# Quantco/tabmat

Hardware: AMD Instinct MI355X
Metric: SplitMatrix.sandwich GFLOP/s + effective HBM GB/s, 10M×1k mixed (higher is better)
Workload: dtype f64; 1 GPU; SplitMatrix.sandwich: dense128 + csr512@5% + cats(256,96,32), 10000000 rows/GPU, p=1024, float64 (BASELINE configs[3]); rows_per_gpu=10000000, p=1024, launch=eager, collective=none

## Files before the change

### tabmat_amd/csrc/cat.hip

```cpp
#include <algorithm>

#include "common.hpp"
#include "reduce.hpp"

namespace tmh {

__global__ void fill_i32_kernel(int32_t *p, int64_t n, int32_t v) {
    int64_t i = (int64_t)blockIdx.x * blockDim.x + threadIdx.x;
    if (i < n) p[i] = v;
}

__global__ void scatter_iota_i32_kernel(int32_t *map, const int32_t *cols, int64_t n_cols) {
    int64_t i = (int64_t)blockIdx.x * blockDim.x + threadIdx.x;
    if (i < n_cols) map[cols[i]] = (int32_t)i;
}

int build_col_map(int32_t *map, int64_t m, const int32_t *cols, int64_t n_cols, hipStream_t st) {
    if (m > 0) {
        hipLaunchKernelGGL(fill_i32_kernel, dim3((unsigned)ceil_div(m, 256)), dim3(256), 0, st, map,
                           m, -1);
        TM_LAUNCH_CHECK();
    }
    if (n_cols > 0) {
        hipLaunchKernelGGL(scatter_iota_i32_kernel, dim3((unsigned)ceil_div(n_cols, 256)),
// ... 5 lines not shown

template <typename F, bool TWO>
__global__ __launch_bounds__(1024) void hist_lds_kernel(
    const int32_t *__restrict__ ci, const int32_t *__restrict__ cj, const F *__restrict__ w,
    const int32_t *__restrict__ rows, int64_t n_iter, int64_t rows_per_block, int drop_i,
    int drop_j, int i_ncol, int j_ncol, int ti, const int32_t *__restrict__ col_map,
    F *__restrict__ ws, int64_t stride) {
    extern __shared__ __attribute__((aligned(16))) unsigned char smem_raw[];
    lds_acc_t *bins = reinterpret_cast<lds_acc_t *>(smem_raw);
    const int part = blockIdx.y;
    const int i0 = part * ti;
    const int i1 = min(i0 + ti, i_ncol);
    const int nbins = TWO ? (i1 - i0) * j_ncol : (i1 - i0);
    for (int b = threadIdx.x; b < nbins; b += blockDim.x) bins[b] = 0.0;
    __syncthreads();

    const int64_t t0 = (int64_t)blockIdx.x * rows_per_block;
    const int64_t t1 = min(t0 + rows_per_block, n_iter);
    int64_t tbeg = t0;
    if (!TWO && rows == nullptr && (t0 & 3) == 0 &&
        ((reinterpret_cast<uintptr_t>(ci) | reinterpret_cast<uintptr_t>(w)) & 15) == 0) {
        typedef int i4 __attribute__((ext_vector_type(4)));
        const int64_t nvec = (t1 - t0) / 4;
        for (int64_t q = threadIdx.x; q < nvec; q += blockDim.x) {
            const int64_t k = t0 + q * 4;
            const i4 cc = *reinterpret_cast<const i4 *>(ci + k);
            F ww[4];
#pragma unroll
            for (int e = 0; e < 4; ++e) ww[e] = w[k + e];
#pragma unroll
            for (int e = 0; e < 4; ++e) {
                const int c = cc[e] - drop_i;
                if (c >= i0 && c < i1 && !(col_map && col_map[c] < 0)) atomic_add(&bins[c - i0], (lds_acc_t)ww[e]);
            }
        }
        tbeg = t0 + nvec * 4;
    }
    for (int64_t t = tbeg + threadIdx.x; t < t1; t += blockDim.x) {
        const int64_t k = rows ? (int64_t)rows[t] : t;
        const int c = ci[k] - drop_i;
        if (c < i0 || c >= i1) continue;
        if (TWO) {
            const int c2 = cj[k] - drop_j;
            if (c2 < 0) continue;
            atomic_add(&bins[(c - i0) * j_ncol + c2], (lds_acc_t)w[k]);
        } else {
            if (col_map && col_map[c] < 0) continue;
            atomic_add(&bins[c - i0], (lds_acc_t)w[k]);
        }
    }
    __syncthreads();
    F *dst = ws + ((int64_t)part * gridDim.x + blockIdx.x) * stride;
    for (int b = threadIdx.x; b < nbins; b += blockDim.x) dst[b] = (F)bins[b];
}

template <typename F, bool TWO>
__global__ __launch_bounds__(256) void hist_global_kernel(
    const int32_t *__restrict__ ci, const int32_t *__restrict__ cj, const F *__restrict__ w,
    const int32_t *__restrict__ rows, int64_t n_iter, int drop_i, int drop_j, int j_ncol,
    const int32_t *__restrict__ col_map, F *__restrict__ out) {
    const int64_t stride = (int64_t)gridDim.x * blockDim.x;
    for (int64_t t = (int64_t)blockIdx.x * blockDim.x + threadIdx.x; t < n_iter; t += stride) {
        const int64_t k = rows ? (int64_t)rows[t] : t;
        const int c = ci[k] - drop_i;
        if (c < 0) continue;
        if (TWO) {
// ... 1203 lines not shown
    cs->total = off;
    return TM_OK;
}

template <typename F>
static int run_multi_cat_dense(const void *const *h_codes, const int64_t *h_ncols,
                               const int32_t *h_drop, int n_cats, int64_t n, const F *d, const F *M,
                               int64_t m, int order_f, F *out, hipStream_t st,
                               const int32_t *rows = nullptr, int64_t n_rows = 0) {
    CatSet cs;
    int rc = make_catset(h_codes, h_ncols, h_drop, n_cats, &cs);
    if (rc) return rc;
    const int64_t total = (int64_t)cs.total * m;
    if (total == 0) return TM_OK;
    if (rows != nullptr) n = n_rows;
    if (n == 0) {
        TM_HIP(hipMemsetAsync(out, 0, sizeof(F) * (size_t)total, st));
        return TM_OK;
    }
    {
        constexpr int VEC = MCW_VEC;
        constexpr int TJW = 16 * VEC;
        const size_t tile_b = ((sizeof(lds_acc_t) * (size_t)cs.total * TJW + 15) / 16) * 16;
        const size_t lds_w = tile_b + (size_t)16 * MCW_RS * (sizeof(F) + (size_t)n_cats * sizeof(int));
        if (!order_f && n_cats <= 8 && m >= VEC && m % VEC == 0 &&
            (reinterpret_cast<uintptr_t>(M) & 15) == 0 && lds_w <= 150 * 1024 &&
            (int64_t)cs.total * TJW * (int64_t)sizeof(lds_acc_t) < (1ll << 30)) {
            const int64_t n_parts = ceil_div(m, TJW);
            const int64_t stride = (int64_t)cs.total * TJW;
            int64_t nblk = std::max<int64_t>(1, tune("catdense_rounds", 1) * NUM_CU / n_parts);
            nblk = std::min<int64_t>(nblk, std::max<int64_t>(1, ceil_div(n, 4096)));
            const int64_t rpb = ceil_div(ceil_div(n, nblk), MCW_RS) * MCW_RS;
            nblk = ceil_div(n, rpb);
            const size_t tmp_bytes = ((sizeof(F) * (size_t)(n_parts * stride) + 255) / 256) * 256;
            void *wsv = nullptr;
            rc = get_workspace(tmp_bytes + sizeof(F) * (size_t)(n_parts * nblk * stride) + 256, &wsv, st);
            if (rc) return rc;
            F *tmp = reinterpret_cast<F *>(wsv);
            F *ws = reinterpret_cast<F *>(reinterpret_cast<char *>(wsv) + tmp_bytes);
            auto gow = [&](auto kern) -> int {
                TM_HIP(hipFuncSetAttribute(reinterpret_cast<const void *>(kern),
                                           hipFuncAttributeMaxDynamicSharedMemorySize, (int)lds_w));
                prof_begin(st);
                const int nw_dflt = (sizeof(F) == 8 && tile_b > 64 * 1024) ? 8 : 16;
                const int nw = (int)std::min<int64_t>(16, std::max<int64_t>(4, tune("catdense_waves", nw_dflt)));
                hipLaunchKernelGGL(kern, dim3((unsigned)nblk, (unsigned)n_parts), dim3(nw * 64), lds_w, st,
                                   cs, d, M, n, m, rpb, ws, stride, rows, wg_log_ptr());
                prof_end(st);
                TM_LAUNCH_CHECK();
                return TM_OK;
            };
            if (n_cats == 1) rc = gow(&multi_cat_dense_wide_kernel<F, 1>);
            else if (n_cats == 2) rc = gow(&multi_cat_dense_wide_kernel<F, 2>);
            else if (n_cats == 3) rc = gow(&multi_cat_dense_wide_kernel<F, 3>);
            else if (n_cats == 4) rc = gow(&multi_cat_dense_wide_kernel<F, 4>);
            else if (n_cats == 5) rc = gow(&multi_cat_dense_wide_kernel<F, 5>);
            else if (n_cats == 6) rc = gow(&multi_cat_dense_wide_kernel<F, 6>);
            else if (n_cats == 7) rc = gow(&multi_cat_dense_wide_kernel<F, 7>);
            else rc = gow(&multi_cat_dense_wide_kernel<F, 8>);
            if (rc) return rc;
            rc = launch_reduce_partials<F>(ws, stride, (int)nblk, (int)n_parts, tmp, n_parts * stride,
                                           false, st);
            if (rc) return rc;
            hipLaunchKernelGGL((multi_cat_untile_kernel<F>), dim3((unsigned)ceil_div(total, 256)),
                               dim3(256), 0, st, tmp, (int64_t)cs.total, m, TJW, out);
            TM_LAUNCH_CHECK();
            return TM_OK;
        }
    }
    if (rows != nullptr) {
        set_error("multi_cat_dense: the row-list form needs the wide-load path");
        return TM_EUNSUPPORTED;
    }
    int TJ = 64;
    while (TJ > 1 && sizeof(lds_acc_t) * (size_t)cs.total * TJ > HIST_LDS_MAX) TJ >>= 1;
    while (TJ > 1 && TJ / 2 >= m) TJ >>= 1;
    if (sizeof(lds_acc_t) * (size_t)cs.total * TJ > HIST_LDS_MAX) {
        set_error("multi_cat_dense: %d stacked categories exceed the LDS tile", cs.total);
        return TM_EUNSUPPORTED;
    }
    const int64_t n_parts = ceil_div(m, TJ);
    const int64_t stride = (int64_t)cs.total * TJ;
    const size_t lds = sizeof(lds_acc_t) * (size_t)stride;
    int64_t nblk = std::max<int64_t>(1, NUM_CU / n_parts);
    nblk = std::min<int64_t>(nblk, std::max<int64_t>(1, ceil_div(n, 4096)));
    const int64_t rpb = ceil_div(n, nblk);
    nblk = ceil_div(n, rpb);
    const size_t tmp_bytes = ((sizeof(F) * (size_t)(n_parts * stride) + 255) / 256) * 256;
    void *wsv = nullptr;
    rc = get_workspace(tmp_bytes + sizeof(F) * (size_t)(n_parts * nblk * stride) + 256, &wsv, st);
    if (rc) return rc;
    F *tmp = reinterpret_cast<F *>(wsv);
    F *ws = reinterpret_cast<F *>(reinterpret_cast<char *>(wsv) + tmp_bytes);
    auto go = [&](auto kern) -> int {
        if (lds > 48 * 1024)
            TM_HIP(hipFuncSetAttribute(reinterpret_cast<const void *>(kern),
                                       hipFuncAttributeMaxDynamicSharedMemorySize, (int)lds));
        prof_begin(st);
        hipLaunchKernelGGL(kern, dim3((unsigned)nblk, (unsigned)n_parts), dim3(1024), lds, st, cs, d,
                           M, n, m, rpb, ws, stride);
// ... 132 lines not shown
}

template <typename F>
static int run_multi_cat_sparse_ent(const void *const *h_codes, const int64_t *h_ncols, const int32_t *h_drop,
                                    int n_cats, int64_t n, const F *d, const F *vals, const unsigned short *meta,
                                    const unsigned *bstart, int64_t mk, F *out, hipStream_t st,
                                    const unsigned *packed = nullptr, int64_t n_slots = 0) {
    CatSet cs;
    int rc = make_catset(h_codes, h_ncols, h_drop, n_cats, &cs);
    if (rc) return rc;
    const int64_t total = (int64_t)cs.total * mk;
    if (total == 0) return TM_OK;
    if (n == 0) {
        TM_HIP(hipMemsetAsync(out, 0, sizeof(F) * (size_t)total, st));
        return TM_OK;
    }
    TM_REQUIRE(mk % 16 == 0 && n_cats >= 1 && n_cats <= 8, "kernel columns in groups of 16, 1 .. 8 categoricals");
    TM_REQUIRE(n < (1ll << 28), "at most 2^28 - 1 rows per block");
    constexpr int GC = 32;
    const int64_t stride = (int64_t)cs.total * GC;
    const size_t lds = ((sizeof(lds_acc_t) * (size_t)cs.total * (GC + 1) + 15) / 16) * 16;
    if (lds > HIST_LDS_MAX) {
        set_error("multi_cat_sparse_ent: %d stacked categories exceed the LDS tile", cs.total);
        return TM_EUNSUPPORTED;
    }
    const int nw = (int)std::min<int64_t>(16, std::max<int64_t>(4, tune("catsparse_waves", 16)));
    const int n_groups = (int)(mk / 16);
    const int n_pairs = (n_groups + 1) / 2;
    const int64_t n_slabs = ceil_div(n, 64);
    int64_t nblk = std::max<int64_t>(1, tune("catsparse_rounds", 1) * NUM_CU / n_pairs);
    nblk = std::min<int64_t>(nblk, n_slabs);
    const int64_t spb = ceil_div(n_slabs, nblk);
    nblk = ceil_div(n_slabs, spb);
    const size_t tmp_bytes = ((sizeof(F) * (size_t)(n_pairs * stride) + 255) / 256) * 256;
    void *wsv = nullptr;
    rc = get_workspace(tmp_bytes + sizeof(F) * (size_t)((int64_t)n_pairs * nblk * stride) + 256, &wsv, st);
    if (rc) return rc;
    F *tmp = reinterpret_cast<F *>(wsv);
    F *ws = reinterpret_cast<F *>(reinterpret_cast<char *>(wsv) + tmp_bytes);
    auto kern = n_cats == 1   ? &multi_cat_sparse_ent_kernel<F, 1>
                : n_cats == 2 ? &multi_cat_sparse_ent_kernel<F, 2>
                : n_cats == 3 ? &multi_cat_sparse_ent_kernel<F, 3>
                : n_cats == 4 ? &multi_cat_sparse_ent_kernel<F, 4>
                : n_cats == 5 ? &multi_cat_sparse_ent_kernel<F, 5>
                : n_cats == 6 ? &multi_cat_sparse_ent_kernel<F, 6>
                : n_cats == 7 ? &multi_cat_sparse_ent_kernel<F, 7>
                              : &multi_cat_sparse_ent_kernel<F, 8>;
    TM_REQUIRE(packed == nullptr || (n_cats <= 3 && cs.total < 1023), "packed codes: at most 3 categoricals, 1022 levels");
    const int ncw = packed != nullptr ? 1 : n_cats;
    const size_t lds_staged = lds + (size_t)nw * 64 * (sizeof(F) + 4 * (size_t)ncw);
    const double fill = (double)n_slots / ((double)std::max(n_groups, 1) * (double)n_slabs);
    if (tune("catsparse_staged", 1) != 0 && lds_staged <= 156 * 1024 &&
        fill >= (double)tune("catsparse_staged_fill", 44)) {
        using KS = void (*)(CatSet, const F *, const F *, const unsigned short *, const unsigned *, int, int64_t, int64_t,
                            int64_t, F *, int64_t, const unsigned *, int);
        KS ks = nullptr;
        if (packed != nullptr) {
            ks = n_cats == 1 ? &multi_cat_sparse_ent_staged_kernel<F, 1, true>
                 : n_cats == 2 ? &multi_cat_sparse_ent_staged_kernel<F, 2, true>
                               : &multi_cat_sparse_ent_staged_kernel<F, 3, true>;
        } else {
            ks = n_cats == 1   ? &multi_cat_sparse_ent_staged_kernel<F, 1, false>
                 : n_cats == 2 ? &multi_cat_sparse_ent_staged_kernel<F, 2, false>
                 : n_cats == 3 ? &multi_cat_sparse_ent_staged_kernel<F, 3, false>
                 : n_cats == 4 ? &multi_cat_sparse_ent_staged_kernel<F, 4, false>
                 : n_cats == 5 ? &multi_cat_sparse_ent_staged_kernel<F, 5, false>
                 : n_cats == 6 ? &multi_cat_sparse_ent_staged_kernel<F, 6, false>
                 : n_cats == 7 ? &multi_cat_sparse_ent_staged_kernel<F, 7, false>
                               : &multi_cat_sparse_ent_staged_kernel<F, 8, false>;
        }
        if (lds_staged > 48 * 1024)
            TM_HIP(hipFuncSetAttribute(reinterpret_cast<const void *>(ks),
                                       hipFuncAttributeMaxDynamicSharedMemorySize, (int)lds_staged));
        prof_begin(st);
        hipLaunchKernelGGL(ks, dim3((unsigned)nblk, (unsigned)n_pairs), dim3(nw * 64), lds_staged, st, cs, d, vals,
                           meta, bstart, n_groups, n, n_slabs, spb, ws, stride, packed, (int)lds);
        prof_end(st);
        TM_LAUNCH_CHECK();
    } else {
        if (lds > 48 * 1024)
            TM_HIP(hipFuncSetAttribute(reinterpret_cast<const void *>(kern),
                                       hipFuncAttributeMaxDynamicSharedMemorySize, (int)lds));
        prof_begin(st);
        hipLaunchKernelGGL(kern, dim3((unsigned)nblk, (unsigned)n_pairs), dim3(nw * 64), lds, st, cs, d, vals, meta,
                           bstart, n_groups, n, n_slabs, spb, ws, stride, packed);
        prof_end(st);
        TM_LAUNCH_CHECK();
    }
    rc = launch_reduce_partials<F>(ws, stride, (int)nblk, n_pairs, tmp, (int64_t)n_pairs * stride, false, st);
    if (rc) return rc;
    hipLaunchKernelGGL((multi_cat_untile_kernel<F>), dim3((unsigned)ceil_div(total, 256)), dim3(256), 0, st, tmp,
                       (int64_t)cs.total, mk, GC, out);
    TM_LAUNCH_CHECK();
    return TM_OK;
}

}

using namespace tmh;

#define TM_CHECK_COMMON(nn) \
    TM_REQUIRE((nn) >= 0, "negative size")

extern "C" {

int tm_cat_transpose_matvec_f32(const int32_t *codes, int64_t n, int64_t n_cols, int drop_first,
                                const float *v, const int32_t *rows, int64_t n_rows,
                                const int32_t *cols, int64_t n_cols_sel, float *out, void *stream) {
    TM_CHECK_COMMON(n);
    return run_cat_tmv<float>(codes, n, n_cols, drop_first, v, rows, n_rows, cols, n_cols_sel, out,
                              as_stream(stream));
}
int tm_cat_transpose_matvec_f64(const int32_t *codes, int64_t n, int64_t n_cols, int drop_first,
                                const double *v, const int32_t *rows, int64_t n_rows,
                                const int32_t *cols, int64_t n_cols_sel, double *out,
                                void *stream) {
    TM_CHECK_COMMON(n);
    return run_cat_tmv<double>(codes, n, n_cols, drop_first, v, rows, n_rows, cols, n_cols_sel,
                               out, as_stream(stream));
}

int tm_cat_matvec_f32(const int32_t *codes, int64_t n, int64_t n_cols, int drop_first,
                      const float *v, const int32_t *cols, int64_t n_cols_sel, float *out,
                      void *stream) {
    TM_CHECK_COMMON(n);
    return run_cat_matvec<float>(codes, n, n_cols, drop_first, v, cols, n_cols_sel, out,
                                 as_stream(stream));
// ... 298 lines not shown
```

### tabmat_amd/csrc/reduce.hpp

```cpp
#pragma once
#include "common.hpp"

namespace tmh {

template <typename F, bool ACCUMULATE, int NW>
__global__ __launch_bounds__(NW * 64) void reduce_partials_kernel(const F *__restrict__ ws,
                                                                  int64_t stride, int nb,
                                                                  F *__restrict__ out,
                                                                  int64_t out_elems) {
    __shared__ double red[NW][64];
    const int lane = threadIdx.x & 63;
    const int wave = threadIdx.x >> 6;
    const int64_t e = (int64_t)blockIdx.x * 64 + lane;
    const int part = blockIdx.y;
    double acc = 0.0;
    if (e < stride) {
        const F *p = ws + ((int64_t)part * nb) * stride + e;
        for (int b = wave; b < nb; b += NW) acc += (double)p[(int64_t)b * stride];
    }
    red[wave][lane] = acc;
    __syncthreads();
    if (wave == 0 && e < stride) {
        const int64_t o = (int64_t)part * stride + e;
        if (o < out_elems) {
// ... 2 lines not shown
            for (int w = 0; w < NW; w += 4)
                s += (red[w][lane] + red[w + 1][lane]) + (red[w + 2][lane] + red[w + 3][lane]);
            if (ACCUMULATE)
                out[o] += (F)s;
            else
                out[o] = (F)s;
        }
    }
}

template <typename F>
inline int launch_reduce_partials(const F *ws, int64_t stride, int nb, int n_parts, F *out,
                                  int64_t out_elems, bool accumulate, hipStream_t st) {
    dim3 grid((unsigned)ceil_div(stride, 64), (unsigned)n_parts);
    const bool small = (int64_t)grid.x * grid.y < 1024 && nb > 16;
    if (small) {
        if (accumulate)
            hipLaunchKernelGGL((reduce_partials_kernel<F, true, 16>), grid, dim3(1024), 0, st, ws,
                               stride, nb, out, out_elems);
        else
            hipLaunchKernelGGL((reduce_partials_kernel<F, false, 16>), grid, dim3(1024), 0, st, ws,
                               stride, nb, out, out_elems);
    } else if (accumulate) {
        hipLaunchKernelGGL((reduce_partials_kernel<F, true, 4>), grid, dim3(256), 0, st, ws, stride,
                           nb, out, out_elems);
    } else {
        hipLaunchKernelGGL((reduce_partials_kernel<F, false, 4>), grid, dim3(256), 0, st, ws, stride,
                           nb, out, out_elems);
    }
    TM_LAUNCH_CHECK();
    return TM_OK;
}

__global__ void fill_i32_kernel(int32_t *p, int64_t n, int32_t v);
__global__ void scatter_iota_i32_kernel(int32_t *map, const int32_t *cols, int64_t n_cols);

int build_col_map(int32_t *map, int64_t m, const int32_t *cols, int64_t n_cols, hipStream_t st);

}
```

### tabmat_amd/csrc/sparse_blocks.hip

```cpp
#include <algorithm>

#include "common.hpp"
#include "reduce.hpp"

namespace tmh {

constexpr int KB_WAVES = 16;
constexpr int KB_TS = 128;

template <typename F>
__global__ void blocks_assemble_kernel(const F *__restrict__ tiles, int n_out, F *__restrict__ out) {
    const int j = blockIdx.x * blockDim.x + threadIdx.x;
    const int i = blockIdx.y;
    if (i >= n_out || j >= n_out) return;
    const int hi = max(i, j), lo = min(i, j);
    const int I = hi / KB_TS, J = lo / KB_TS;
    const int part = I * (I + 1) / 2 + J;
    out[(int64_t)i * n_out + j] = tiles[(int64_t)part * KB_TS * KB_TS + (hi % KB_TS) * KB_TS + (lo % KB_TS)];
}

constexpr int KB_FLAG_REP_A = 1 << 16;
constexpr int KB_FLAG_REP_B = 1 << 17;

template <typename F, bool U8, bool D12 = false>
__global__ __launch_bounds__(KB_WAVES * 64) void sparse_sandwich_blocks_kernel(
    const F *__restrict__ data, const int32_t *__restrict__ ind, const int32_t *__restrict__ cptr,
    int64_t n, int64_t nnz1, const int32_t *__restrict__ blocks, const int4 *__restrict__ wg_tab,
    const F *__restrict__ d, int max_nb, F *__restrict__ ws, WgLogBuf *__restrict__ wglog) {
    constexpr int TS = KB_TS;
    const unsigned long long t_begin = wg_log_begin(wglog);
    extern __shared__ __attribute__((aligned(16))) unsigned char smem_raw[];
    lds_acc_t *tile = reinterpret_cast<lds_acc_t *>(smem_raw);
    const int4 w = wg_tab[2 * blockIdx.x], x = wg_tab[2 * blockIdx.x + 1];
    const int part = __builtin_amdgcn_readfirstlane(w.x), slot = __builtin_amdgcn_readfirstlane(w.y);
    const int b0 = __builtin_amdgcn_readfirstlane(w.z), b1 = __builtin_amdgcn_readfirstlane(w.w);
    const int bfull = __builtin_amdgcn_readfirstlane(x.x);
    int wfull = __builtin_amdgcn_readfirstlane(x.y);
    {
        const int nwv = (int)(blockDim.x >> 6);
        if (nwv != KB_WAVES) {
            wfull = (wfull * nwv + KB_WAVES / 2) / KB_WAVES;
            if (bfull > b0) wfull = max(wfull, 1);
            if (b1 > bfull) wfull = min(wfull, nwv - 1);
            if (bfull == b0) wfull = 0;
            if (b1 == bfull) wfull = nwv;
        }
    }
    int I = (int)((sqrtf(8.0f * (float)part + 1.0f) - 1.0f) * 0.5f);
    while ((I + 1) * (I + 2) / 2 <= part) ++I;
    while (I * (I + 1) / 2 > part) --I;
    const int J = part - I * (I + 1) / 2;
    const int i0 = I * TS, j0 = J * TS;
// ... 131 lines not shown
        };
        auto run_tile = [&](auto diag_c) {
            if (wave < wfull) run_list(diag_c, std::true_type{}, b0, bfull, 0, wfull);
            else run_list(diag_c, std::false_type{}, bfull, b1, wfull, (int)(blockDim.x >> 6) - wfull);
        };
        if (I == J) run_tile(std::true_type{});
        else run_tile(std::false_type{});
    }
    __syncthreads();
    if (threadIdx.x == 0) wg_log_end(wglog, t_begin, WG_K2);
    F *dst = ws + ((int64_t)part * max_nb + slot) * (TS * TS);
    for (int b = threadIdx.x; b < TS * TS; b += blockDim.x) {
        const int r = b / TS, c = b % TS;
        dst[b] = (F)tile[r * TS + (c ^ ((r & 15) << 3))];
    }
}

template <typename F, bool U8 = false, bool D12 = false>
static int run_sparse_sandwich_blocks(const F *data, const int32_t *ind, const int32_t *cptr, int64_t n,
                                      int64_t m, int64_t nnz, const int32_t *blocks, const int32_t *wg_tab,
                                      int n_wg, int max_nb, const F *d, F *out, hipStream_t st) {
    if (m == 0) return TM_OK;
    if (n == 0 || nnz == 0 || n_wg == 0) {
        TM_HIP(hipMemsetAsync(out, 0, sizeof(F) * (size_t)(m * m), st));
        return TM_OK;
    }
    constexpr int TS = KB_TS;
    const int nchunk = (int)ceil_div(m, TS);
    const int n_parts = nchunk * (nchunk + 1) / 2;
    TM_REQUIRE(nnz < (1ll << 31) && n < (1ll << 29), "sparse block too large for the block-list sandwich");
    TM_REQUIRE(!D12 || n < (1ll << 24), "12-byte block descriptors hold 24 bits of row");
    TM_REQUIRE(max_nb >= 1 && n_wg >= 1, "empty workgroup table");
    const size_t lds = sizeof(lds_acc_t) * (size_t)(TS * TS);
    const size_t tmp_bytes = (sizeof(F) * (size_t)n_parts * TS * TS + 255) / 256 * 256;
    const size_t ws_bytes = sizeof(F) * (size_t)n_parts * (size_t)max_nb * TS * TS;
    void *wsv = nullptr;
    int rc = get_workspace(tmp_bytes + ws_bytes + 256, &wsv, st);
    if (rc) return rc;
    F *tmp = reinterpret_cast<F *>(wsv);
    F *ws = reinterpret_cast<F *>(reinterpret_cast<char *>(wsv) + tmp_bytes);
    TM_HIP(hipMemsetAsync(ws, 0, ws_bytes, st));
    auto kern = &sparse_sandwich_blocks_kernel<F, U8, D12>;
    TM_HIP(hipFuncSetAttribute(reinterpret_cast<const void *>(kern),
                               hipFuncAttributeMaxDynamicSharedMemorySize, (int)lds));
    prof_begin(st);
    const int kb_waves = (int)std::min<int64_t>(KB_WAVES, std::max<int64_t>(2, tune("k2b_waves", KB_WAVES)));
    hipLaunchKernelGGL(kern, dim3((unsigned)n_wg), dim3(kb_waves * 64), lds, st, data, ind, cptr, n, nnz - 1,
                       blocks, reinterpret_cast<const int4 *>(wg_tab), d,
                       max_nb, ws, wg_log_ptr());
    prof_end(st);
    TM_LAUNCH_CHECK();
    rc = launch_reduce_partials<F>(ws, (int64_t)TS * TS, max_nb, n_parts, tmp, (int64_t)n_parts * TS * TS,
                                   false, st);
    if (rc) return rc;
    hipLaunchKernelGGL((blocks_assemble_kernel<F>), dim3((unsigned)ceil_div(m, 64), (unsigned)m), dim3(64),
                       0, st, tmp, (int)m, out);
    TM_LAUNCH_CHECK();
    return TM_OK;
}

}

extern "C" {

int tm_sparse_sandwich_blocks_f32(const float *cm_data, const int32_t *cm_indices, const int32_t *cptr,
                                  int64_t n, int64_t m, int64_t nnz, const int32_t *blocks,
                                  const int32_t *wg_tab, int n_wg, int max_nb, const float *d, float *out,
                                  void *stream) {
    return tmh::run_sparse_sandwich_blocks<float>(cm_data, cm_indices, cptr, n, m, nnz, blocks, wg_tab, n_wg,
                                                  max_nb, d, out, tmh::as_stream(stream));
}
int tm_sparse_sandwich_blocks_f64(const double *cm_data, const int32_t *cm_indices, const int32_t *cptr,
                                  int64_t n, int64_t m, int64_t nnz, const int32_t *blocks,
                                  const int32_t *wg_tab, int n_wg, int max_nb, const double *d, double *out,
                                  void *stream) {
    return tmh::run_sparse_sandwich_blocks<double>(cm_data, cm_indices, cptr, n, m, nnz, blocks, wg_tab, n_wg,
                                                   max_nb, d, out, tmh::as_stream(stream));
}

int tm_sparse_sandwich_blocks_u8_f32(const float *cm_data, const uint8_t *cm_col8, const int32_t *cptr,
                                     int64_t n, int64_t m, int64_t nnz, const int32_t *blocks,
                                     const int32_t *wg_tab, int n_wg, int max_nb, const float *d, float *out,
                                     void *stream) {
    return tmh::run_sparse_sandwich_blocks<float, true>(cm_data, reinterpret_cast<const int32_t *>(cm_col8), cptr, n, m,
                                                        nnz, blocks, wg_tab, n_wg, max_nb, d, out,
                                                        tmh::as_stream(stream));
}
int tm_sparse_sandwich_blocks_u8_f64(const double *cm_data, const uint8_t *cm_col8, const int32_t *cptr,
                                     int64_t n, int64_t m, int64_t nnz, const int32_t *blocks,
                                     const int32_t *wg_tab, int n_wg, int max_nb, const double *d, double *out,
                                     void *stream) {
// ... 24 lines not shown
```

### tabmat_amd/csrc/sparse_ent.hip

```cpp
#include "common.hpp"
#include "reduce.hpp"

namespace tmh {

constexpr int EN_R = 64;
constexpr int EN_C = 16;
constexpr int EN_NW = 16;
constexpr int EN_THREADS = EN_NW * 64;
constexpr int EN_W = 128;
constexpr int EN_B = 16;
constexpr int EN_SB = 64;

template <typename F>
struct EnLds {
    static constexpr int ROWB = EN_W * (int)sizeof(F);
    static constexpr int SLABB = EN_R * ROWB;
    static constexpr int SCR_OFF = ROWB + 2 * SLABB;
    static constexpr int CS_OFF = SCR_OFF + EN_NW * EN_SB * 16;
    static constexpr int TOTAL = CS_OFF + EN_NW * EN_C * (int)sizeof(double);
};

constexpr int EN_CVGPR = 24;
#define EN_LD "40"

// ... 286 lines not shown
#endif
    }
    while (w < ns) end_slab();
    wait_loads(std::integral_constant<int, 0>{});
#if defined(EN_PROF)
    if (prof != nullptr && lane == 0) {
        long long *o = prof + (((int64_t)blockIdx.z * gridDim.y + blockIdx.y) * gridDim.x + blockIdx.x) * (EN_NW * 8) + wave * 8;
        o[0] = pt_a; o[1] = pt_p; o[2] = pt_x; o[3] = pt_b; o[4] = pt_bar; o[5] = pt_n; o[6] = clock64() - pt_start; o[7] = ns;
    }
#endif

    if (active) {
        F *dst = ws + (((int64_t)blockIdx.y * gridDim.x + blockIdx.x) * n_groups + group) * (EN_C * EN_W);
        static_for<EN_C>([&](auto jc) {
            constexpr int j = decltype(jc)::value;
            if constexpr (sizeof(F) == 8) {
                const u4 o = u4{en_read_acc<4 * j>(), en_read_acc<4 * j + 1>(), en_read_acc<4 * j + 2>(),
                                en_read_acc<4 * j + 3>()};
                *reinterpret_cast<u4 *>(dst + j * EN_W + 2 * lane) = o;
            } else {
                typedef unsigned u2 __attribute__((ext_vector_type(2)));
                const u2 o = u2{en_read_acc<2 * j>(), en_read_acc<2 * j + 1>()};
                *reinterpret_cast<u2 *>(dst + j * EN_W + 2 * lane) = o;
            }
        });
        if constexpr (CSUM) {
            if (blockIdx.y == 0 && lane < EN_C)
                ws_csum[(int64_t)blockIdx.x * (n_groups * EN_C) + group * EN_C + lane] = (F)cs_lds[lane];
        }
    }
}

template <typename F>
__global__ void en_untile_kernel(const F *__restrict__ tmp, int64_t m, int64_t nB, F *__restrict__ out) {
    const int64_t e = (int64_t)blockIdx.x * blockDim.x + threadIdx.x;
    if (e >= m * nB) return;
    const int64_t i = e / nB, j = e % nB;
    out[e] = tmp[((j / EN_W) * m + i) * EN_W + (j % EN_W)];
}

template <typename F>
__global__ void en_csum_kernel(const F *__restrict__ part, int nblk, int64_t m, F *__restrict__ csum) {
    const int64_t c = (int64_t)blockIdx.x * blockDim.x + threadIdx.x;
    if (c >= m) return;
    double a = 0.0;
    for (int b = 0; b < nblk; ++b) a += (double)part[(int64_t)b * m + c];
    csum[c] = (F)a;
}

template <typename F>
static int run_csr_dense_ent(const F *vals, const uint16_t *meta, const uint32_t *bstart, int64_t n, int64_t m,
                             const F *B, int64_t r, const F *d, F *out, F *colsum, hipStream_t st) {
    const int64_t nB = r;
    const int64_t total = m * nB;
    if (total == 0) return TM_OK;
    constexpr int VEC = 16 / (int)sizeof(F);
    if ((reinterpret_cast<uintptr_t>(B) & 15) != 0 || r % VEC != 0 || nB < VEC) {
        set_error("tm_csr_dense_sandwich_ent: B must be C-ordered with 16-byte aligned rows");
        return TM_EUNSUPPORTED;
    }
    if (m % EN_C != 0) {
        set_error("tm_csr_dense_sandwich_ent: m must be a multiple of tm_ent_group_cols()");
        return TM_EINVAL;
    }
    if (n >= (1ll << 28)) {
        set_error("tm_csr_dense_sandwich_ent: at most 2^28 - 1 rows per block (work in row parts)");
        return TM_EUNSUPPORTED;
    }
    const int64_t n_slabs = ceil_div(n, EN_R);
    const int n_groups = (int)(m / EN_C);
    const int n_parts = (int)ceil_div(nB, EN_W);
    const int nz = (int)ceil_div(n_groups, EN_NW);
    const bool want_csum = colsum != nullptr;
    if (n_slabs == 0) {
        TM_HIP(hipMemsetAsync(out, 0, sizeof(F) * (size_t)total, st));
        if (want_csum) TM_HIP(hipMemsetAsync(colsum, 0, sizeof(F) * (size_t)m, st));
        return TM_OK;
    }
    int64_t nblk = std::max<int64_t>(1, tune("ent_rounds", 1) * NUM_CU / ((int64_t)n_parts * nz));
    nblk = std::min<int64_t>(nblk, n_slabs);
    const int64_t spb = ceil_div(n_slabs, nblk);
    nblk = ceil_div(n_slabs, spb);
    const int64_t stride = m * EN_W;
    const size_t tmp_bytes = (sizeof(F) * (size_t)(n_parts * stride) + 255) / 256 * 256;
    const size_t part_bytes = (sizeof(F) * (size_t)((int64_t)n_parts * nblk * stride) + 255) / 256 * 256;
    const size_t csum_bytes = ((want_csum ? sizeof(F) * (size_t)(nblk * m) : 0) + 255) / 256 * 256 + 256;
    void *wsv = nullptr;
    int rc = get_workspace(tmp_bytes + part_bytes + csum_bytes + 256, &wsv, st);
    if (rc) return rc;
    F *tmp = reinterpret_cast<F *>(wsv);
    F *ws = reinterpret_cast<F *>(reinterpret_cast<char *>(wsv) + tmp_bytes);
    F *ws_csum = reinterpret_cast<F *>(reinterpret_cast<char *>(wsv) + tmp_bytes + part_bytes);
    const size_t lds = (size_t)EnLds<F>::TOTAL;
    auto kern = want_csum ? &csr_dense_ent_kernel<F, true> : &csr_dense_ent_kernel<F, false>;
    TM_HIP(hipFuncSetAttribute(reinterpret_cast<const void *>(kern),
                               hipFuncAttributeMaxDynamicSharedMemorySize, (int)lds));
    prof_begin(st);
    hipLaunchKernelGGL(kern, dim3((unsigned)nblk, (unsigned)n_parts, (unsigned)nz), dim3(EN_THREADS), lds, st,
                       vals, meta, bstart, n_groups, n_slabs, spb, B, n, r, (int)nB, d, ws, ws_csum,
                       reinterpret_cast<long long *>((uintptr_t)tune("ent_prof", 0)));
    prof_end(st);
    TM_LAUNCH_CHECK();
    rc = launch_reduce_partials<F>(ws, stride, (int)nblk, n_parts, tmp, n_parts * stride, false, st);
    if (rc) return rc;
    hipLaunchKernelGGL((en_untile_kernel<F>), dim3((unsigned)ceil_div(total, 256)), dim3(256), 0, st, tmp, m,
                       nB, out);
    TM_LAUNCH_CHECK();
    if (want_csum) {
        hipLaunchKernelGGL((en_csum_kernel<F>), dim3((unsigned)ceil_div(m, 256)), dim3(256), 0, st, ws_csum,
                           (int)nblk, m, colsum);
        TM_LAUNCH_CHECK();
    }
    return TM_OK;
}

}

extern "C" {
int tm_ent_rows(void) { return tmh::EN_R; }
int tm_ent_group_cols(void) { return tmh::EN_C; }
int tm_ent_batch_slots(void) { return tmh::EN_B; }

int tm_csr_dense_sandwich_ent_f32(const float *vals, const uint16_t *meta, const uint32_t *bstart, int64_t n,
                                  int64_t m, const float *B, int64_t r, const float *d, float *out,
                                  float *colsum, void *stream) {
    return tmh::run_csr_dense_ent<float>(vals, meta, bstart, n, m, B, r, d, out, colsum, tmh::as_stream(stream));
}
int tm_csr_dense_sandwich_ent_f64(const double *vals, const uint16_t *meta, const uint32_t *bstart, int64_t n,
                                  int64_t m, const double *B, int64_t r, const double *d, double *out,
                                  double *colsum, void *stream) {
    return tmh::run_csr_dense_ent<double>(vals, meta, bstart, n, m, B, r, d, out, colsum, tmh::as_stream(stream));
}
}
```

### tabmat_amd/csrc/syrk_i8.hip

```cpp
#include <algorithm>
#include <cmath>

#include "common.hpp"

#if defined(I8_NO_SB)
#define I8_SB
#else
#define I8_SB __builtin_amdgcn_sched_barrier(0)
#endif
#if defined(I8_TRACE)
#define I8_STAMP(k)                                                                                     \
    do {                                                                                                \
        if (blockIdx.x == 0 && lane == 0 && trace_it >= 8 && trace_it < 12)                             \
            trace_buf[((trace_it - 8) * 4 + wave) * 8 + (k)] = __builtin_readcyclecounter();            \
    } while (0)
#else
#define I8_STAMP(k)
#endif
namespace tmh {

constexpr int I8_W = 128;
constexpr int I8_T = 36;
constexpr int I8_ND = 5;
constexpr int I8_WLO = 2;
// ... 156 lines not shown
    }
    sigma[i] = s;
    rscale[i] = r;
}

template <bool CSUM, bool CEN, bool TV = false>
__global__ __launch_bounds__(I8_THREADS) __attribute__((amdgpu_waves_per_eu(1, 1)))
void syrk_i8_kernel(const double *__restrict__ X, int64_t ldx, int64_t n, int64_t m, const double *__restrict__ d,
                    const double *__restrict__ sigma, const I8Info *__restrict__ info, int n_items,
                    unsigned *__restrict__ counter, double *__restrict__ part, double *__restrict__ colsum,
                    const double *__restrict__ center, const double *__restrict__ v = nullptr,
                    double *__restrict__ xtv = nullptr) {
    if (info->flag != 0) return;
    __shared__ __attribute__((aligned(16))) unsigned char planes[I8_PLANES];
    __shared__ __attribute__((aligned(16))) unsigned char raw[3 * I8_RAWBUF];
    __shared__ double dl[3 * I8_HS];
    __shared__ double vl[TV ? 3 * I8_HS : 1];
    __shared__ unsigned slot_mem[4];
    unsigned *slot = slot_mem;
#if defined(I8_TRACE)
    unsigned long long *trace_buf = reinterpret_cast<unsigned long long *>(reinterpret_cast<char *>(counter) - 256 + 2560);
    int trace_it = 0;
#endif

    const int tid = threadIdx.x;
    const int lane = tid & 63;
    const int wave = __builtin_amdgcn_readfirstlane(tid >> 6);
    const int cl = lane & 15, rq = lane >> 4;

    unsigned idL = blockIdx.x;
    int hL = 0;
    unsigned idNext;
    if (tid == 0) *slot = gridDim.x + atomicAdd(counter, 1u);
    __syncthreads();
    idNext = __builtin_amdgcn_readfirstlane(*slot);
    bool pending = false;

    using C0 = std::integral_constant<int, 0>;
    using C1 = std::integral_constant<int, 1>;
    double dreg = 0.0, vreg = 0.0;
    const int dma_voff = lane * 2 < m ? lane * 16 : 0x7ffffff0;
    auto issue_half = [&](int rb) -> unsigned {
        const unsigned id = idL;
        const int64_t tb = (int64_t)id * I8_ITEM_ROWS + (int64_t)hL * I8_HS;
        const int64_t left = min((n - tb) * ldx * 8, (int64_t)I8_HS * ldx * 8);
        const uint64_t xb = (uint64_t)(uintptr_t)(X + tb * ldx);
        const unsigned xlo = __builtin_amdgcn_readfirstlane((unsigned)xb);
        const unsigned xhi = __builtin_amdgcn_readfirstlane((unsigned)(xb >> 32));
        const unsigned nbytes = __builtin_amdgcn_readfirstlane(
            left <= 0 ? 0u : (left > 0xFFFFFFFFll ? 0xFFFFFFFFu : (unsigned)left));
        const i8_rsrc_t rs = i8_rsrc(reinterpret_cast<const void *>((uintptr_t)(((uint64_t)xhi << 32) | xlo)), nbytes);
        if (wave == 0 && lane < I8_HS) dreg = tb + lane < n ? d[tb + lane] : 0.0;
        if constexpr (TV) {
            if (wave == 0 && lane < I8_HS) vreg = tb + lane < n ? v[tb + lane] : 0.0;
        }
#if !defined(I8_ABLATE_NO_DMA)
#pragma unroll
        for (int j = 0; j < 8; ++j)
            i8_dma16(rs, raw + rb * I8_RAWBUF + (8 * wave + j) * I8_RAWSTR, (int)((8 * wave + j) * ldx * 8) + dma_voff);
#endif
        if (++hL == 2 * I8_CPI) {
            hL = 0;
            idL = idNext;
            if (tid == 0) *slot = gridDim.x + atomicAdd(counter, 1u);
            pending = true;
        }
// ... 412 lines not shown

int run_syrk_i8_panel(const double *X, int64_t ldx, int64_t n, int64_t m, const double *d, const double *colmax,
                      double *out, int64_t ldo, double *colsum, int *history, hipStream_t st, const double *center,
                      const double *v, double *xtv) {
    TM_REQUIRE((v == nullptr) == (xtv == nullptr), "v and xtv go together");
    TM_REQUIRE(v == nullptr || colsum == nullptr, "X' d and X' v are not built into one int8 kernel");
    TM_REQUIRE(n >= 0 && m >= 0, "negative shape");
    TM_REQUIRE(ldx >= m && ldo >= m, "row strides");
    TM_REQUIRE(m == 0 || syrk_co_ok(X, m), "the int8 syrk takes a 16-byte aligned C-ordered f64 block of <= 128 columns");
    if (m == 0) return TM_OK;
    if (n == 0) {
        TM_HIP(hipMemset2DAsync(out, sizeof(double) * (size_t)ldo, 0, sizeof(double) * (size_t)m, (size_t)m, st));
        if (colsum) TM_HIP(hipMemsetAsync(colsum, 0, sizeof(double) * (size_t)m, st));
        if (xtv) TM_HIP(hipMemsetAsync(xtv, 0, sizeof(double) * (size_t)m, st));
        return TM_OK;
    }
    if (colsum) TM_HIP(hipMemsetAsync(colsum, 0, sizeof(double) * (size_t)m, st));
    if (xtv) TM_HIP(hipMemsetAsync(xtv, 0, sizeof(double) * (size_t)m, st));
    const int64_t n_items64 = ceil_div(n, I8_ITEM_ROWS);
    TM_REQUIRE(n_items64 < (1ll << 31), "too many rows");
    const int n_items = (int)n_items64;
    const int grid = (int)std::max<int64_t>(1, std::min<int64_t>(n_items, tune("i8_grid", NUM_CU)));
    const size_t part_bytes = sizeof(double) * (size_t)grid * I8_T * 256;
    const size_t own_bytes = (4096 + part_bytes + 255) / 256 * 256;
    void *wsv = nullptr;
    int rc = get_workspace(own_bytes + syrk_co_ws_bytes(), &wsv, st);
    if (rc) return rc;
    char *wb = reinterpret_cast<char *>(wsv);
    I8Info *info = reinterpret_cast<I8Info *>(wb);
    unsigned *counter = reinterpret_cast<unsigned *>(wb + 256);
    double *sigma = reinterpret_cast<double *>(wb + 512);
    double *rscale = reinterpret_cast<double *>(wb + 512 + 1024);
    double *part = reinterpret_cast<double *>(wb + 4096);
    TM_HIP(hipMemsetAsync(wb, 0, 4096 + part_bytes, st));
    const int sgrid = (int)std::min<int64_t>(4 * NUM_CU, ceil_div(n, 1024));
    hipLaunchKernelGGL(i8_screen_kernel, dim3((unsigned)sgrid), dim3(256), 0, st, d, n, info);
    hipLaunchKernelGGL(i8_scale_kernel, dim3(1), dim3(I8_W), 0, st, colmax, (int)m, n, info, sigma, rscale, history);
    TM_LAUNCH_CHECK();
    prof_begin(st);
    auto go = [&](auto kern) {
        hipLaunchKernelGGL(kern, dim3((unsigned)grid), dim3(I8_THREADS), 0, st, X, ldx, n, m, d, sigma, info, n_items,
                           counter, part, colsum, center, v, xtv);
    };
    if (v) {
        if (center) go(syrk_i8_kernel<false, true, true>);
        else go(syrk_i8_kernel<false, false, true>);
    } else if (center) {
        if (colsum) go(syrk_i8_kernel<true, true>);
        else go(syrk_i8_kernel<false, true>);
    } else {
        if (colsum) go(syrk_i8_kernel<true, false>);
        else go(syrk_i8_kernel<false, false>);
    }
    prof_end(st);
    TM_LAUNCH_CHECK();
    hipLaunchKernelGGL(syrk_i8_finish_kernel, dim3(I8_T, 4), dim3(64, 16), 0, st, part, grid, (int)m, rscale, info,
                       out, ldo);
    hipLaunchKernelGGL(i8_envelope_kernel, dim3(1), dim3(I8_W), 0, st, out, ldo, colmax, (int)m, n, info, history);
    TM_LAUNCH_CHECK();
    prof_hold(true);
    rc = run_syrk_co_flagged(X, ldx, n, m, d, out, ldo, colsum, &info->flag, wb + own_bytes, st, center, v, xtv);
    prof_hold(false);
    if (rc == TM_OK && history != nullptr) {
        hipLaunchKernelGGL(i8_record_diag_kernel, dim3(1), dim3(I8_W), 0, st, out, ldo, (int)m, history);
        TM_LAUNCH_CHECK();
    }
    return rc;
// ... 50 lines not shown
```

Before: 1047 GB/s.

## Fuse partial reduction with untile/assemble and drop workspace memsets

Replaces the two-step reduce-partials plus untile/assemble launches in the categorical, sparse-entry, CSR-dense and sparse-blocks sandwich paths with a single finish kernel that sums partials and writes directly into the output layout. The sparse-blocks path gains a masked variant that reads only the partial slots that workgroups actually wrote, which lets it skip the large workspace memset. The int8 syrk kernel now zeroes its own partial slab instead of relying on a host memset. A vectorized nontemporal load path is also added for the two-categorical histogram kernel. Risk: the masked finish depends on the workgroup table covering every written slot, and the output mapping logic is new.

```diff
diff --git a/tabmat_amd/csrc/cat.hip b/tabmat_amd/csrc/cat.hip
--- a/tabmat_amd/csrc/cat.hip
+++ b/tabmat_amd/csrc/cat.hip
@@ -61,6 +61,25 @@
             for (int e = 0; e < 4; ++e) {
                 const int c = cc[e] - drop_i;
                 if (c >= i0 && c < i1 && !(col_map && col_map[c] < 0)) atomic_add(&bins[c - i0], (lds_acc_t)ww[e]);
+            }
+        }
+        tbeg = t0 + nvec * 4;
+    }
+    if (TWO && rows == nullptr && (t0 & 3) == 0 &&
+        ((reinterpret_cast<uintptr_t>(ci) | reinterpret_cast<uintptr_t>(cj) | reinterpret_cast<uintptr_t>(w)) & 15) == 0) {
+        typedef int i4 __attribute__((ext_vector_type(4)));
+        const int64_t nvec = (t1 - t0) / 4;
+        for (int64_t q = threadIdx.x; q < nvec; q += blockDim.x) {
+            const int64_t k = t0 + q * 4;
+            const i4 cc = __builtin_nontemporal_load(reinterpret_cast<const i4 *>(ci + k));
+            const i4 cc2 = __builtin_nontemporal_load(reinterpret_cast<const i4 *>(cj + k));
+            F ww[4];
+#pragma unroll
+            for (int e = 0; e < 4; ++e) ww[e] = w[k + e];
+#pragma unroll
+            for (int e = 0; e < 4; ++e) {
+                const int c = cc[e] - drop_i, c2 = cc2[e] - drop_j;
+                if (c >= i0 && c < i1 && c2 >= 0) atomic_add(&bins[(c - i0) * j_ncol + c2], (lds_acc_t)ww[e]);
             }
         }
         tbeg = t0 + nvec * 4;
@@ -1330,12 +1349,10 @@
             nblk = std::min<int64_t>(nblk, std::max<int64_t>(1, ceil_div(n, 4096)));
             const int64_t rpb = ceil_div(ceil_div(n, nblk), MCW_RS) * MCW_RS;
             nblk = ceil_div(n, rpb);
-            const size_t tmp_bytes = ((sizeof(F) * (size_t)(n_parts * stride) + 255) / 256) * 256;
             void *wsv = nullptr;
-            rc = get_workspace(tmp_bytes + sizeof(F) * (size_t)(n_parts * nblk * stride) + 256, &wsv, st);
+            rc = get_workspace(sizeof(F) * (size_t)(n_parts * nblk * stride) + 256, &wsv, st);
             if (rc) return rc;
-            F *tmp = reinterpret_cast<F *>(wsv);
-            F *ws = reinterpret_cast<F *>(reinterpret_cast<char *>(wsv) + tmp_bytes);
+            F *ws = reinterpret_cast<F *>(wsv);
             auto gow = [&](auto kern) -> int {
                 TM_HIP(hipFuncSetAttribute(reinterpret_cast<const void *>(kern),
                                            hipFuncAttributeMaxDynamicSharedMemorySize, (int)lds_w));
@@ -1357,13 +1374,7 @@
             else if (n_cats == 7) rc = gow(&multi_cat_dense_wide_kernel<F, 7>);
             else rc = gow(&multi_cat_dense_wide_kernel<F, 8>);
             if (rc) return rc;
-            rc = launch_reduce_partials<F>(ws, stride, (int)nblk, (int)n_parts, tmp, n_parts * stride,
-                                           false, st);
-            if (rc) return rc;
-            hipLaunchKernelGGL((multi_cat_untile_kernel<F>), dim3((unsigned)ceil_div(total, 256)),
-                               dim3(256), 0, st, tmp, (int64_t)cs.total, m, TJW, out);
-            TM_LAUNCH_CHECK();
-            return TM_OK;
+            return launch_finish_partials<F>(ws, stride, (int)nblk, (int)n_parts, FinishMapPanel{TJW, m}, out, st);
         }
     }
     if (rows != nullptr) {
@@ -1562,12 +1573,10 @@
     nblk = std::min<int64_t>(nblk, n_slabs);
     const int64_t spb = ceil_div(n_slabs, nblk);
     nblk = ceil_div(n_slabs, spb);
-    const size_t tmp_bytes = ((sizeof(F) * (size_t)(n_pairs * stride) + 255) / 256) * 256;
     void *wsv = nullptr;
-    rc = get_workspace(tmp_bytes + sizeof(F) * (size_t)((int64_t)n_pairs * nblk * stride) + 256, &wsv, st);
+    rc = get_workspace(sizeof(F) * (size_t)((int64_t)n_pairs * nblk * stride) + 256, &wsv, st);
     if (rc) return rc;
-    F *tmp = reinterpret_cast<F *>(wsv);
-    F *ws = reinterpret_cast<F *>(reinterpret_cast<char *>(wsv) + tmp_bytes);
+    F *ws = reinterpret_cast<F *>(wsv);
     auto kern = n_cats == 1   ? &multi_cat_sparse_ent_kernel<F, 1>
                 : n_cats == 2 ? &multi_cat_sparse_ent_kernel<F, 2>
                 : n_cats == 3 ? &multi_cat_sparse_ent_kernel<F, 3>
@@ -1617,12 +1626,7 @@
         prof_end(st);
         TM_LAUNCH_CHECK();
     }
-    rc = launch_reduce_partials<F>(ws, stride, (int)nblk, n_pairs, tmp, (int64_t)n_pairs * stride, false, st);
-    if (rc) return rc;
-    hipLaunchKernelGGL((multi_cat_untile_kernel<F>), dim3((unsigned)ceil_div(total, 256)), dim3(256), 0, st, tmp,
-                       (int64_t)cs.total, mk, GC, out);
-    TM_LAUNCH_CHECK();
-    return TM_OK;
+    return launch_finish_partials<F>(ws, stride, (int)nblk, n_pairs, FinishMapPanel{GC, mk}, out, st);
 }
 
 }
diff --git a/tabmat_amd/csrc/reduce.hpp b/tabmat_amd/csrc/reduce.hpp
--- a/tabmat_amd/csrc/reduce.hpp
+++ b/tabmat_amd/csrc/reduce.hpp
@@ -58,6 +58,157 @@
     return TM_OK;
 }
 
+
+struct FinishMapPanel {
+    int W;
+    int64_t ncols;
+    __device__ void place(int part, int64_t e, int64_t &o, int64_t &o2) const {
+        const int64_t row = e / W, col = (int64_t)part * W + (e % W);
+        o = col < ncols ? row * ncols + col : -1;
+        o2 = -1;
+    }
+};
+
+struct FinishMapTriTiles {
+    int TS;
+    int n_out;
+    __device__ void place(int part, int64_t e, int64_t &o, int64_t &o2) const {
+        int I = 0;
+        while ((I + 1) * (I + 2) / 2 <= part) ++I;
+        const int J = part - I * (I + 1) / 2;
+        const int r = (int)(e / TS), c = (int)(e % TS);
+        const int hi = I * TS + r, lo = J * TS + c;
+        o = o2 = -1;
+        if (hi < n_out && lo < n_out && (I != J || c <= r)) {
+            o = (int64_t)hi * n_out + lo;
+            if (hi != lo) o2 = (int64_t)lo * n_out + hi;
+        }
+    }
+};
+
+constexpr int FINISH_MASK_WORDS = 64;
+
+template <typename F, int NW, typename Map>
+__global__ __launch_bounds__(NW * 64) void finish_partials_kernel(const F *__restrict__ ws, int64_t stride, int nb,
+                                                                  Map map, F *__restrict__ out) {
+    __shared__ double red[NW][64];
+    const int lane = threadIdx.x & 63;
+    const int wave = threadIdx.x >> 6;
+    const int64_t e = (int64_t)blockIdx.x * 64 + lane;
+    const int part = blockIdx.y;
+    double acc = 0.0;
+    if (e < stride) {
+        const F *p = ws + ((int64_t)part * nb) * stride + e;
+        for (int b = wave; b < nb; b += NW) acc += (double)p[(int64_t)b * stride];
+    }
+    red[wave][lane] = acc;
+    __syncthreads();
+    if (wave == 0 && e < stride) {
+        double s = 0.0;
+#pragma unroll
+        for (int w = 0; w < NW; w += 4)
+            s += (red[w][lane] + red[w + 1][lane]) + (red[w + 2][lane] + red[w + 3][lane]);
+        int64_t o, o2;
+        map.place(part, e, o, o2);
+        if (o >= 0) out[o] = (F)s;
+        if (o2 >= 0) out[o2] = (F)s;
+    }
+}
+
+template <typename F, int NW, int G, typename Map>
+__global__ __launch_bounds__(NW * 64) void finish_partials_masked_kernel(const F *__restrict__ ws, int64_t stride,
+                                                                         int nb, Map map, F *__restrict__ out,
+                                                                         const int4 *__restrict__ wg_tab, int n_wg) {
+    constexpr int SLOTS = FINISH_MASK_WORDS * 32;
+    __shared__ double red[G][NW][64];
+    __shared__ unsigned mask[FINISH_MASK_WORDS];
+    __shared__ int first[FINISH_MASK_WORDS + 1];
+    __shared__ int list[SLOTS];
+    const int lane = threadIdx.x & 63;
+    const int wave = threadIdx.x >> 6;
+    const int part = blockIdx.y;
+    const int64_t e0 = (int64_t)blockIdx.x * (64 * G) + lane;
+    const F *p = ws + ((int64_t)part * nb) * stride + e0;
+    double acc[G];
+#pragma unroll
+    for (int g = 0; g < G; ++g) acc[g] = 0.0;
+    for (int base = 0; base < nb; base += SLOTS) {
+        const int top = min(nb, base + SLOTS);
+        __syncthreads();
+        if (threadIdx.x < FINISH_MASK_WORDS) mask[threadIdx.x] = 0u;
+        __syncthreads();
+        for (int w = threadIdx.x; w < n_wg; w += NW * 64) {
+            const int4 t = wg_tab[2 * w];
+            if (t.x == part && t.y >= base && t.y < top) atomicOr(&mask[(t.y - base) >> 5], 1u << ((t.y - base) & 31));
+        }
+        __syncthreads();
+        if (threadIdx.x == 0) {
+            int c = 0;
+            for (int w = 0; w < FINISH_MASK_WORDS; ++w) {
+                first[w] = c;
+                c += __popc(mask[w]);
+            }
+            first[FINISH_MASK_WORDS] = c;
+        }
+        __syncthreads();
+        if (threadIdx.x < FINISH_MASK_WORDS) {
+            unsigned m = mask[threadIdx.x];
+            int k = first[threadIdx.x];
+            while (m) {
+                const int bit = __ffs(m) - 1;
+                list[k++] = base + (int)threadIdx.x * 32 + bit;
+                m &= m - 1;
+            }
+        }
+        __syncthreads();
+        const int cnt = first[FINISH_MASK_WORDS];
+#pragma unroll 4
+        for (int k = wave; k < cnt; k += NW) {
+            const F *q = p + (int64_t)list[k] * stride;
+#pragma unroll
+            for (int g = 0; g < G; ++g) acc[g] += (double)q[64 * g];
+        }
+    }
+#pragma unroll
+    for (int g = 0; g < G; ++g) red[g][wave][lane] = acc[g];
+    __syncthreads();
+    if (wave < G) {
+        double s = 0.0;
+#pragma unroll
+        for (int w = 0; w < NW; w += 4)
+            s += (red[wave][w][lane] + red[wave][w + 1][lane]) + (red[wave][w + 2][lane] + red[wave][w + 3][lane]);
+        int64_t o, o2;
+        map.place(part, e0 + 64 * wave, o, o2);
+        if (o >= 0) out[o] = (F)s;
+        if (o2 >= 0) out[o2] = (F)s;
+    }
+}
+
+template <typename F, typename Map>
+inline int launch_finish_partials(const F *ws, int64_t stride, int nb, int n_parts, Map map, F *out, hipStream_t st) {
+    dim3 grid((unsigned)ceil_div(stride, 64), (unsigned)n_parts);
+    const bool small = (int64_t)grid.x * grid.y < 1024 && nb > 16;
+    if (small)
+        hipLaunchKernelGGL((finish_partials_kernel<F, 16, Map>), grid, dim3(1024), 0, st, ws, stride, nb, map, out);
+    else
+        hipLaunchKernelGGL((finish_partials_kernel<F, 4, Map>), grid, dim3(256), 0, st, ws, stride, nb, map, out);
+    TM_LAUNCH_CHECK();
+    return TM_OK;
+}
+
+template <typename F, typename Map>
+inline int launch_finish_partials_masked(const F *ws, int64_t stride, int nb, int n_parts, Map map, F *out,
+                                         const int32_t *wg_tab, int n_wg, hipStream_t st) {
+    constexpr int NW = 4, G = 4;
+    static_assert(G <= NW, "wave g finishes run g");
+    TM_REQUIRE(stride % (64 * G) == 0, "finish: tile size");
+    dim3 grid((unsigned)(stride / (64 * G)), (unsigned)n_parts);
+    hipLaunchKernelGGL((finish_partials_masked_kernel<F, NW, G, Map>), grid, dim3(NW * 64), 0, st, ws, stride, nb, map,
+                       out, reinterpret_cast<const int4 *>(wg_tab), n_wg);
+    TM_LAUNCH_CHECK();
+    return TM_OK;
+}
+
 __global__ void fill_i32_kernel(int32_t *p, int64_t n, int32_t v);
 __global__ void scatter_iota_i32_kernel(int32_t *map, const int32_t *cols, int64_t n_cols);
 
diff --git a/tabmat_amd/csrc/sparse_blocks.hip b/tabmat_amd/csrc/sparse_blocks.hip
--- a/tabmat_amd/csrc/sparse_blocks.hip
+++ b/tabmat_amd/csrc/sparse_blocks.hip
@@ -7,17 +7,6 @@
 
 constexpr int KB_WAVES = 16;
 constexpr int KB_TS = 128;
-
-template <typename F>
-__global__ void blocks_assemble_kernel(const F *__restrict__ tiles, int n_out, F *__restrict__ out) {
-    const int j = blockIdx.x * blockDim.x + threadIdx.x;
-    const int i = blockIdx.y;
-    if (i >= n_out || j >= n_out) return;
-    const int hi = max(i, j), lo = min(i, j);
-    const int I = hi / KB_TS, J = lo / KB_TS;
-    const int part = I * (I + 1) / 2 + J;
-    out[(int64_t)i * n_out + j] = tiles[(int64_t)part * KB_TS * KB_TS + (hi % KB_TS) * KB_TS + (lo % KB_TS)];
-}
 
 constexpr int KB_FLAG_REP_A = 1 << 16;
 constexpr int KB_FLAG_REP_B = 1 << 17;
@@ -215,14 +204,11 @@
     TM_REQUIRE(!D12 || n < (1ll << 24), "12-byte block descriptors hold 24 bits of row");
     TM_REQUIRE(max_nb >= 1 && n_wg >= 1, "empty workgroup table");
     const size_t lds = sizeof(lds_acc_t) * (size_t)(TS * TS);
-    const size_t tmp_bytes = (sizeof(F) * (size_t)n_parts * TS * TS + 255) / 256 * 256;
     const size_t ws_bytes = sizeof(F) * (size_t)n_parts * (size_t)max_nb * TS * TS;
     void *wsv = nullptr;
-    int rc = get_workspace(tmp_bytes + ws_bytes + 256, &wsv, st);
+    int rc = get_workspace(ws_bytes + 256, &wsv, st);
     if (rc) return rc;
-    F *tmp = reinterpret_cast<F *>(wsv);
-    F *ws = reinterpret_cast<F *>(reinterpret_cast<char *>(wsv) + tmp_bytes);
-    TM_HIP(hipMemsetAsync(ws, 0, ws_bytes, st));
+    F *ws = reinterpret_cast<F *>(wsv);
     auto kern = &sparse_sandwich_blocks_kernel<F, U8, D12>;
     TM_HIP(hipFuncSetAttribute(reinterpret_cast<const void *>(kern),
                                hipFuncAttributeMaxDynamicSharedMemorySize, (int)lds));
@@ -233,13 +219,8 @@
                        max_nb, ws, wg_log_ptr());
     prof_end(st);
     TM_LAUNCH_CHECK();
-    rc = launch_reduce_partials<F>(ws, (int64_t)TS * TS, max_nb, n_parts, tmp, (int64_t)n_parts * TS * TS,
-                                   false, st);
-    if (rc) return rc;
-    hipLaunchKernelGGL((blocks_assemble_kernel<F>), dim3((unsigned)ceil_div(m, 64), (unsigned)m), dim3(64),
-                       0, st, tmp, (int)m, out);
-    TM_LAUNCH_CHECK();
-    return TM_OK;
+    return launch_finish_partials_masked<F>(ws, (int64_t)TS * TS, max_nb, n_parts, FinishMapTriTiles{TS, (int)m}, out,
+                                            wg_tab, n_wg, st);
 }
 
 }
diff --git a/tabmat_amd/csrc/sparse_ent.hip b/tabmat_amd/csrc/sparse_ent.hip
--- a/tabmat_amd/csrc/sparse_ent.hip
+++ b/tabmat_amd/csrc/sparse_ent.hip
@@ -342,14 +342,6 @@
 }
 
 template <typename F>
-__global__ void en_untile_kernel(const F *__restrict__ tmp, int64_t m, int64_t nB, F *__restrict__ out) {
-    const int64_t e = (int64_t)blockIdx.x * blockDim.x + threadIdx.x;
-    if (e >= m * nB) return;
-    const int64_t i = e / nB, j = e % nB;
-    out[e] = tmp[((j / EN_W) * m + i) * EN_W + (j % EN_W)];
-}
-
-template <typename F>
 __global__ void en_csum_kernel(const F *__restrict__ part, int nblk, int64_t m, F *__restrict__ csum) {
     const int64_t c = (int64_t)blockIdx.x * blockDim.x + threadIdx.x;
     if (c >= m) return;
@@ -392,15 +384,13 @@
     const int64_t spb = ceil_div(n_slabs, nblk);
     nblk = ceil_div(n_slabs, spb);
     const int64_t stride = m * EN_W;
-    const size_t tmp_bytes = (sizeof(F) * (size_t)(n_parts * stride) + 255) / 256 * 256;
     const size_t part_bytes = (sizeof(F) * (size_t)((int64_t)n_parts * nblk * stride) + 255) / 256 * 256;
     const size_t csum_bytes = ((want_csum ? sizeof(F) * (size_t)(nblk * m) : 0) + 255) / 256 * 256 + 256;
     void *wsv = nullptr;
-    int rc = get_workspace(tmp_bytes + part_bytes + csum_bytes + 256, &wsv, st);
+    int rc = get_workspace(part_bytes + csum_bytes + 256, &wsv, st);
     if (rc) return rc;
-    F *tmp = reinterpret_cast<F *>(wsv);
-    F *ws = reinterpret_cast<F *>(reinterpret_cast<char *>(wsv) + tmp_bytes);
-    F *ws_csum = reinterpret_cast<F *>(reinterpret_cast<char *>(wsv) + tmp_bytes + part_bytes);
+    F *ws = reinterpret_cast<F *>(wsv);
+    F *ws_csum = reinterpret_cast<F *>(reinterpret_cast<char *>(wsv) + part_bytes);
     const size_t lds = (size_t)EnLds<F>::TOTAL;
     auto kern = want_csum ? &csr_dense_ent_kernel<F, true> : &csr_dense_ent_kernel<F, false>;
     TM_HIP(hipFuncSetAttribute(reinterpret_cast<const void *>(kern),
@@ -411,11 +401,8 @@
                        reinterpret_cast<long long *>((uintptr_t)tune("ent_prof", 0)));
     prof_end(st);
     TM_LAUNCH_CHECK();
-    rc = launch_reduce_partials<F>(ws, stride, (int)nblk, n_parts, tmp, n_parts * stride, false, st);
+    rc = launch_finish_partials<F>(ws, stride, (int)nblk, n_parts, FinishMapPanel{EN_W, nB}, out, st);
     if (rc) return rc;
-    hipLaunchKernelGGL((en_untile_kernel<F>), dim3((unsigned)ceil_div(total, 256)), dim3(256), 0, st, tmp, m,
-                       nB, out);
-    TM_LAUNCH_CHECK();
     if (want_csum) {
         hipLaunchKernelGGL((en_csum_kernel<F>), dim3((unsigned)ceil_div(m, 256)), dim3(256), 0, st, ws_csum,
                            (int)nblk, m, colsum);
diff --git a/tabmat_amd/csrc/syrk_i8.hip b/tabmat_amd/csrc/syrk_i8.hip
--- a/tabmat_amd/csrc/syrk_i8.hip
+++ b/tabmat_amd/csrc/syrk_i8.hip
@@ -212,6 +212,11 @@
     int hL = 0;
     unsigned idNext;
     if (tid == 0) *slot = gridDim.x + atomicAdd(counter, 1u);
+    {
+        double *own = part + (int64_t)blockIdx.x * (I8_T * 256);
+        for (int k = tid; k < I8_T * 256; k += I8_THREADS) own[k] = 0.0;
+        asm volatile("s_waitcnt vmcnt(0)" ::: "memory");
+    }
     __syncthreads();
     idNext = __builtin_amdgcn_readfirstlane(*slot);
     bool pending = false;
@@ -690,7 +695,7 @@
     double *sigma = reinterpret_cast<double *>(wb + 512);
     double *rscale = reinterpret_cast<double *>(wb + 512 + 1024);
     double *part = reinterpret_cast<double *>(wb + 4096);
-    TM_HIP(hipMemsetAsync(wb, 0, 4096 + part_bytes, st));
+    TM_HIP(hipMemsetAsync(wb, 0, 4096, st));
     const int sgrid = (int)std::min<int64_t>(4 * NUM_CU, ceil_div(n, 1024));
     hipLaunchKernelGGL(i8_screen_kernel, dim3((unsigned)sgrid), dim3(256), 0, st, d, n, info);
     hipLaunchKernelGGL(i8_scale_kernel, dim3(1), dim3(I8_W), 0, st, colmax, (int)m, n, info, sigma, rscale, history);
```

Result: no change. 1049 GB/s, median of 6 (+0.2%).
